# Arash-san/YinYang-Game-AlphaZero

Measured on AMD Instinct MI355X. Metric: self-play positions/sec (+ MCTS node-expansions/sec) at 800 sims, 8x8 board, higher is better.
Workload: dtype f16x3; 1 GPU; 8x8 board, 800 sims/move, 4096 concurrent games per GPU, frozen random-init 128x10 net (seed 0), copied boards, reference_quirks=False, staggered start plies; tree_arithmetic=f32 PUCT + u64 bitboards, nn_dtype=f16x3, evaluation_reuse=False, parallelism=episode-sharded x1, lanes_per_gpu=2, hipgraph=True

## Files before the change

include/yy_engine.h:

```cpp
#ifndef YY_ENGINE_H
#define YY_ENGINE_H

#include <stdint.h>

#ifdef __cplusplus
extern "C" {
#endif

#define YY_OK 0
#define YY_E_INVALID (-1)
#define YY_E_UNSUPPORTED (-2)
#define YY_E_NOMEM (-3)
#define YY_E_HIP (-4)
#define YY_E_STATE (-5)
#define YY_E_ARENA (-6)

#define YY_FLAG_ROWCOL 1u
#define YY_FLAG_ALIASED 2u
#define YY_FLAG_REUSE_PASS_VALUE 4u

#define YY_FLAG_REUSE_TRANSPOSITIONS 8u
#define YY_FLAG_KEEP_EVALUATIONS 16u

#define YY_FLAG_EVAL_SYMMETRY 32u
// ... 125 lines not shown
int yy_nn_tower_heads_bf16(const float *planes, const void *weights, const float *bias,
                           void *out_heads, int G, int R, int C, int channels, int n_layers,
                           yy_stream_t stream);

int yy_nn_tower_f32(const float *planes, const void *weights, const float *bias, float *out, int G,
                    int R, int C, int channels, int n_layers, yy_stream_t stream);

int yy_nn_head_finish_bf16(const void *h, int G, int A, int H, const float *w2, const float *b2,
                           float *policy, float *value, yy_stream_t stream);

int yy_nn_tower_f16x3_regs(const float *planes, const void *weights, const void *head_w, const float *bias,
                           float *out, float *out_heads, const int32_t *rows, const int32_t *n_rows, int G,
                           int R, int C, int channels, int n_layers, int weight_exp, int head_exp,
                           int act_exp, yy_stream_t stream);

int yy_nn_tower_g(const float *planes, const void *weights, const void *head_w, const float *bias, const float *head_bias,
                  float *out, float *out_heads, const int32_t *rows, const int32_t *n_rows, int G, int R, int C,
                  int channels, int n_layers, int weight_exp, int head_exp, int act_exp, int nb, int boards, int gate_lo,
                  int gate_hi, int layout, yy_stream_t stream);
int yy_nn_tower_g_forms(int channels, int *nb_out);
int yy_nn_tower_g_relu_check(uint32_t start, uint32_t count, uint32_t *counts, yy_stream_t stream);

int yy_nn_fc_heads_f16x3(const float *feats, const void *wpk, const float *bias, const int32_t *jobs, int n_jobs,
                         float *logits, float *hidden, const int32_t *n_rows, int G, int K, int A, int H,
                         int weight_exp, int act_exp, yy_stream_t stream);

int yy_nn_head_finish_f32(const float *logits, const float *hidden, int G, int A, int H, const float *w2,
                          const float *b2, const int32_t *rows, const int32_t *n_rows, float *policy,
                          float *value, yy_stream_t stream);

int yy_compact_rows(const uint8_t *flags, int G, int32_t *rows, int32_t *n, yy_stream_t stream);

int yy_selfplay_root_noise(uint64_t seed, const int64_t *game_id, const int32_t *ply, const uint8_t *draw,
                           const uint8_t *mask, int G, int A, double alpha, double *noise, yy_stream_t stream);

int yy_selfplay_root_gumbel(uint64_t seed, const int64_t *game_id, const int32_t *ply, int G, int A, float *rows,
                            yy_stream_t stream);

int yy_selfplay_sample_actions(uint64_t seed, const int64_t *game_id, const int32_t *ply,
                               const uint8_t *searching, const double *pi, const uint8_t *mask, int G, int A,
// ... 35 lines not shown
```

yinyang-game-alphazero_amd/_lib.py:

```python
import ctypes as C
import os
import subprocess

_HERE = os.path.dirname(os.path.abspath(__file__))
CSRC = os.path.join(_HERE, "csrc")
SO = os.path.join(CSRC, "libyy_hip.so")
HEADER = os.path.normpath(os.path.join(_HERE, "..", "include", "yy_engine.h"))

YY_OK = 0
YY_E_ARENA = -6
FLAG_ROWCOL = 1
FLAG_ALIASED = 2
FLAG_REUSE_PASS_VALUE = 4
FLAG_REUSE_TRANSPOSITIONS = 8
FLAG_KEEP_EVALUATIONS = 16
FLAG_EVAL_SYMMETRY = 32
FLAG_FORCED_PLAYOUTS = 64
FLAG_FPU_REDUCTION = 128
FLAG_SOLVER = 256
FLAG_GUMBEL_ROOT = 512
FLAG_GUMBEL_INTERIOR = 1024

HIPCC_FLAGS = ["--offload-arch=gfx950", "-O3", "-std=c++17", "-fPIC", "-shared",
               "-ffp-contract=off", "-fno-fast-math", "-Wall", "-Wno-unused-function"]
# ... 89 lines not shown
    "yy_mcts_shared_counters_ex": [_vp, C.POINTER(C.c_uint64)],
    "yy_nn_bias_act_bf16": [_vp, _vp, _vp, C.c_int64, C.c_int, C.c_int, _vp],
    "yy_nn_tower_bf16": [_vp, _vp, _vp, _vp, C.c_int, C.c_int, C.c_int, C.c_int, C.c_int, _vp],
    "yy_nn_tower_heads_bf16": [_vp, _vp, _vp, _vp, C.c_int, C.c_int, C.c_int, C.c_int, C.c_int, _vp],
    "yy_nn_head_finish_bf16": [_vp, C.c_int, C.c_int, C.c_int, _vp, _vp, _vp, _vp, _vp],
    "yy_nn_tower_f32": [_vp, _vp, _vp, _vp, C.c_int, C.c_int, C.c_int, C.c_int, C.c_int, _vp],
    "yy_nn_head_finish_f32": [_vp, _vp, C.c_int, C.c_int, C.c_int, _vp, _vp, _vp, _vp, _vp, _vp, _vp],
    "yy_compact_rows": [_vp, C.c_int, _vp, _vp, _vp],
    "yy_nn_tower_f16x3_regs": [_vp, _vp, _vp, _vp, _vp, _vp, _vp, _vp, C.c_int, C.c_int, C.c_int, C.c_int, C.c_int, C.c_int, C.c_int,
                               C.c_int, _vp],
    "yy_nn_tower_g_forms": [C.c_int, C.POINTER(C.c_int)],
    "yy_nn_tower_g_relu_check": [C.c_uint32, C.c_uint32, _vp, _vp],
    "yy_nn_tower_g": [_vp, _vp, _vp, _vp, _vp, _vp, _vp, _vp, _vp, C.c_int, C.c_int, C.c_int, C.c_int, C.c_int, C.c_int, C.c_int,
                      C.c_int, C.c_int, C.c_int, C.c_int, C.c_int, C.c_int, _vp],
    "yy_nn_fc_heads_f16x3": [_vp, _vp, _vp, _vp, C.c_int, _vp, _vp, _vp, C.c_int, C.c_int, C.c_int, C.c_int, C.c_int, C.c_int, _vp],
    "yy_selfplay_root_noise": [C.c_uint64, _vp, _vp, _vp, _vp, C.c_int, C.c_int, C.c_double, _vp, _vp],
    "yy_selfplay_root_gumbel": [C.c_uint64, _vp, _vp, C.c_int, C.c_int, _vp, _vp],
    "yy_selfplay_sample_actions": [C.c_uint64, _vp, _vp, _vp, _vp, _vp, C.c_int, C.c_int, C.c_int, _vp, _vp],
    "yy_selfplay_draw_budgets": [C.c_uint64, _vp, _vp, _vp, C.c_int, C.c_double, C.c_int, C.c_int, _vp, _vp, _vp],
    "yy_selfplay_run_create": [_vp, C.POINTER(SelfPlayConfig), C.POINTER(_vp)],
    "yy_selfplay_run_destroy": [_vp],
    "yy_selfplay_run_arm": [_vp, _vp, C.c_int64, C.c_int64, C.c_int64, _vp, _vp, _vp],
    "yy_mcts_step_selfplay": [_vp, _vp, _vp, _vp, _vp, _vp, _vp],
    "yy_selfplay_run_counters": [_vp, _vp, _vp],
    "yy_selfplay_run_examples": [_vp, C.c_int64, C.c_int64, _vp, _vp, _vp, _vp, _vp, _vp],
    "yy_version": [],
}


def exported_symbols():
# ... 25 lines not shown
```

yinyang-game-alphazero_amd/csrc/yy_engine.hip:

```cpp
#include <hip/hip_runtime.h>
#include <math.h>
#include <stdio.h>
#include <string.h>

#include "../../include/yy_engine.h"
#include "yy_bitboard.h"
#include "yy_common.h"
#include "yy_tree.h"

#define YY_VERSION 111

static thread_local char g_err[512] = "";
static int set_err(int code, const char *fmt, const char *a = "", const char *b = "") {
    snprintf(g_err, sizeof g_err, fmt, a, b);
    return code;
}

extern "C" const char *yy_last_error(void) { return g_err; }
extern "C" int yy_tower_set_err(int code, const char *msg) { return set_err(code, "%s%s", msg); }
extern "C" int yy_version(void) { return YY_VERSION; }

static int check_geo(int G, int R, int C) {
    if (G <= 0 || R <= 0 || C <= 0) return set_err(YY_E_INVALID, "non-positive size%s%s");
    if (R > YY_MAX_DIM || C > YY_MAX_DIM || R * C > 64 * YY_MAX_NW)
        return set_err(YY_E_UNSUPPORTED, "board larger than 16x16 / 192 cells%s%s");
// ... 1932 lines not shown
```

yinyang-game-alphazero_amd/csrc/yy_fc_heads.hip:

```cpp
#include <hip/hip_runtime.h>
#include <math.h>
#include <stdint.h>

#include "../../include/yy_engine.h"

typedef __attribute__((ext_vector_type(8))) _Float16 f16x8;
typedef __attribute__((ext_vector_type(2))) _Float16 f16x2;
typedef __attribute__((ext_vector_type(4))) float f32x4;
typedef __attribute__((ext_vector_type(2))) float f32x2;
typedef __attribute__((ext_vector_type(4))) unsigned int u32x4;
typedef __attribute__((ext_vector_type(2))) unsigned int u32x2;

#include "yy_common.h"

namespace fch {

constexpr int KC = 128, RS = 288;

__device__ __forceinline__ void split_pair(const f32x2 a, uint32_t &hi, uint32_t &lo) {
    const f16x2 h = __builtin_convertvector(a, f16x2);
    const f32x2 r = a - __builtin_convertvector(h, f32x2);
    const f16x2 l = __builtin_convertvector(r, f16x2);
    hi = __builtin_bit_cast(uint32_t, h);
    lo = __builtin_bit_cast(uint32_t, l);
// ... 109 lines not shown
    const int o0 = job.out0 + wave * 16 + kg * 4;
    float b[4];
#pragma unroll
    for (int i = 0; i < 4; i++) b[i] = (o0 + i < job.out0 + job.nout) ? bias[boff + o0 + i] : 0.0f;
#pragma unroll
    for (int nb = 0; nb < NBR; nb++) {
        const int row = r0 + nb * 16 + n16;
        if (row < n_live) {
#pragma unroll
            for (int i = 0; i < 4; i++)
                if (o0 + i < job.out0 + job.nout) out[(size_t)row * W + o0 + i] = __builtin_fmaf(acc1[nb][i] + acc2[nb][i], out_scale, b[i]);
        }
    }
}

}

extern "C" int yy_nn_fc_heads_f16x3(const float *feats, const void *wpk, const float *bias, const int32_t *jobs, int n_jobs,
                                    float *logits, float *hidden, const int32_t *n_rows, int G, int K, int A, int H,
                                    int weight_exp, int act_exp, yy_stream_t s) {
    if (G == 0) return YY_OK;
    if (!feats || !wpk || !bias || !jobs || !logits || !hidden || G < 0 || n_jobs < 1 || K < 32 || (K & 31) || A < 1 || H < 1)
        return yy_tower_set_err(YY_E_INVALID, "yy_nn_fc_heads_f16x3: bad argument");
    const float in_scale = ldexpf(1.0f, act_exp), out_scale = ldexpf(1.0f, -(weight_exp + act_exp));
    if (G <= 2048)
        fch::k_fc_heads<32><<<dim3(((G + 31) / 32) * n_jobs), dim3(256), 0, (hipStream_t)s>>>(
            feats, (const unsigned char *)wpk, bias, (const fch::Job *)jobs, n_jobs, logits, hidden, n_rows, G, K, A, H, in_scale, out_scale);
    else
        fch::k_fc_heads<64><<<dim3(((G + 63) / 64) * n_jobs), dim3(256), 0, (hipStream_t)s>>>(
            feats, (const unsigned char *)wpk, bias, (const fch::Job *)jobs, n_jobs, logits, hidden, n_rows, G, K, A, H, in_scale, out_scale);
    if (hipGetLastError() != hipSuccess) return yy_tower_set_err(YY_E_HIP, "yy_nn_fc_heads_f16x3: launch failed");
    return YY_OK;
}
```

yinyang-game-alphazero_amd/csrc/yy_tower_g.hip:

```cpp
#include <hip/hip_runtime.h>
#include <math.h>
#include <stdint.h>

#include <type_traits>

#include "../../include/yy_engine.h"

typedef __attribute__((ext_vector_type(8))) _Float16 f16x8;
typedef __attribute__((ext_vector_type(2))) _Float16 f16x2;
typedef __attribute__((ext_vector_type(4))) float f32x4;
typedef __attribute__((ext_vector_type(2))) float f32x2;
typedef __attribute__((ext_vector_type(4))) unsigned int u32x4;
typedef __attribute__((ext_vector_type(2))) unsigned int u32x2;

#include "yy_common.h"

namespace tg {

template <int NW_, int NB_, int D_, bool RB_> struct Geo {
    static constexpr int NW = NW_, NB = NB_, D = D_, CH = 32 * NW_, NCOL = 16 * NB_;
    static constexpr bool RB = RB_;
    static constexpr int RS = (NW_ >= 3) ? 288 : 160;
    static constexpr int ZERO_OFF = NCOL * RS;
    static constexpr int PART_BYTES = ZERO_OFF + 512;
// ... 179 lines not shown
                                              u32x2 &hi, u32x2 &lo) {
    f32x4 v;
#pragma unroll
    for (int i = 0; i < 4; i++) v[i] = __builtin_fmaf(acc1[i] + acc2[i], acc_scale, bq[i]);
    if (CONV2) v += *(const f32x4 *)res;
#pragma unroll
    for (int i = 0; i < 4; i++) v[i] = RELU(v[i]);
    if (KEEP) *(f32x4 *)res = v;
    uint32_t h01, l01, h23, l23;
    split_pair((f32x2){v[0], v[1]}, h01, l01);
    split_pair((f32x2){v[2], v[3]}, h23, l23);
    hi = (u32x2){h01, h23};
    lo = (u32x2){l01, l23};
}

template <class GEO>
__device__ __forceinline__ void heads_tail(const unsigned char *lds, const unsigned char *head_w, const float *head_bias, float *out_heads,
                                           int g0, int n_live, int C, int cells, int TB, int lane, int wave, float head_scale) {
    constexpr int NW = GEO::NW, NB = GEO::NB, RS = GEO::RS;
    int lane2 = lane;
    asm volatile("" : "+v"(lane2));
    const int n16 = lane2 & 15, kg = lane2 >> 4;
    for (int hm = wave; hm < 4; hm += NW) {
        const int head = hm >> 1, mb = hm & 1;
        f16x8 wh[NW], wl[NW];
#pragma unroll
        for (int kq = 0; kq < NW; kq++) {
            const unsigned char *p = head_w + ((size_t)(hm * NW + kq) * 2) * 1024 + lane2 * 16;
            wh[kq] = __builtin_bit_cast(f16x8, *(const u32x4 *)p);
            wl[kq] = __builtin_bit_cast(f16x8, *(const u32x4 *)(p + 1024));
        }
        const float *hb = head_bias + head * 32 + mb * 16;
        float sb[16];
#pragma unroll
        for (int k = 0; k < 16; k++) {
            sb[k] = hb[k];
            asm volatile("" : "+s"(sb[k]));
        }
        f32x4 b;
#pragma unroll
        for (int i = 0; i < 4; i++) b[i] = kg == 0 ? sb[i] : kg == 1 ? sb[4 + i] : kg == 2 ? sb[8 + i] : sb[12 + i];
#pragma unroll
        for (int nb = 0; nb < NB; nb++) {
            const uint32_t xb = (uint32_t)((nb * 16 + n16) * RS + kg * 16);
            f32x4 h1 = {0.f, 0.f, 0.f, 0.f}, h2 = {0.f, 0.f, 0.f, 0.f};
#pragma unroll
            for (int kq = 0; kq < NW; kq++) {
                const f16x8 xh = __builtin_bit_cast(f16x8, *(const u32x4 *)(lds + xb + kq * 64));
                const f16x8 xl = __builtin_bit_cast(f16x8, *(const u32x4 *)(lds + xb + GEO::PART_BYTES + kq * 64));
                const f32x4 a = __builtin_amdgcn_mfma_f32_16x16x32_f16(wl[kq], xh, h2, 0, 0, 0);
                h1 = __builtin_amdgcn_mfma_f32_16x16x32_f16(wh[kq], xh, h1, 0, 0, 0);
                h2 = __builtin_amdgcn_mfma_f32_16x16x32_f16(wh[kq], xl, a, 0, 0, 0);
            }
            int bd, cell;
            col_board_cell<GEO>(nb * 16 + n16, C, cells, bd, cell);
            const int gb = g0 + bd;
            if (bd < TB && gb < n_live) {
                float *o = out_heads + (((size_t)gb * 2 + head) * 32 + mb * 16 + kg * 4) * cells + cell;
#pragma unroll
                for (int i = 0; i < 4; i++) o[i * cells] = relu_keep_nan(__builtin_fmaf(h1[i] + h2[i], head_scale, b[i]));
            }
        }
    }
}

template <class GEO>
__device__ __forceinline__ void store_activations(const unsigned char *lds, float *out, int g0, int n_live, int C, int cells, int TB,
                                                  float out_scale) {
    constexpr int CH = GEO::CH, RS = GEO::RS, NT = 64 * GEO::NW;
    const int ncol = TB * cells;
    for (int p = threadIdx.x; p < ncol * (CH / 4); p += NT) {
        const int col = p / (CH / 4), ch4 = p % (CH / 4);
        int b, cell;
        col_board_cell<GEO>(col, C, cells, b, cell);
        if (b < TB && g0 + b < n_live) {
            const u32x2 ph = *(const u32x2 *)(lds + col * RS + ch4 * 8);
            const u32x2 pl = *(const u32x2 *)(lds + GEO::PART_BYTES + col * RS + ch4 * 8);
            const f32x2 v01 = join_pair(ph.x, pl.x), v23 = join_pair(ph.y, pl.y);
            *(f32x4 *)(out + ((size_t)(g0 + b) * cells + cell) * CH + ch4 * 4) = (f32x4){v01.x, v01.y, v23.x, v23.y} * out_scale;
        }
    }
}

template <int NW_, int NB_, int D_, bool RB_>
__global__ void __launch_bounds__(64 * NW_, 1)
k_tower_g(const float *__restrict__ planes, const unsigned char *__restrict__ weights, const unsigned char *__restrict__ head_w,
          const float *__restrict__ bias, const float *__restrict__ head_bias, float *__restrict__ out, float *__restrict__ out_heads,
          const int *__restrict__ rows, const int *__restrict__ n_rows, int G, int R, int C, int TB, int n_layers, float in_scale,
          float acc_scale, float head_scale, float out_scale, int gate_lo, int gate_hi) {
    using GEO = Geo<NW_, NB_, D_, RB_>;
    constexpr int NW = GEO::NW, NB = GEO::NB, D = GEO::D, CH = GEO::CH, RS = GEO::RS;
    __shared__ __attribute__((aligned(256))) unsigned char lds[GEO::LDS_BYTES];
    const int n_live = n_rows ? min(*n_rows, G) : G;
    if (n_live <= gate_lo || n_live > gate_hi) return;
    const int g0 = blockIdx.x * TB;
    if (g0 >= n_live) return;
    const int lane = threadIdx.x & 63;
    const int wave = __builtin_amdgcn_readfirstlane(threadIdx.x >> 6);
    const int cells = R * C, n_tower = 9 + 9 * NW * (n_layers - 1), crs = (GEO::RB ? 16 : C) * RS;

    const uint32_t voff = (uint32_t)(wave * 4096 + lane * 16);
    WChunk<2> W[D];
// ... 38 lines not shown
        f32x4 acc1[NB][2], acc2[NB][2];
        __syncthreads();
        run_layer<GEO, true>(acc1, acc2, W, lds, weights, voff, chunk, n_tower, crs, geo);
        __syncthreads();
        epilogue(0, acc1, acc2, std::false_type{}, std::true_type{});
    }
    for (int L = 1; L < n_layers; L++) {
        f32x4 acc1[NB][2], acc2[NB][2];
        __syncthreads();
        run_layer<GEO, false>(acc1, acc2, W, lds, weights, voff, chunk, n_tower, crs, geo);
        __syncthreads();
        if ((L & 1) == 0) epilogue(L, acc1, acc2, std::true_type{}, std::true_type{});
        else epilogue(L, acc1, acc2, std::false_type{}, std::false_type{});
    }
    __syncthreads();
    if (out_heads) heads_tail<GEO>(lds, head_w, head_bias, out_heads, g0, n_live, C, cells, TB, lane, wave, head_scale);
    else store_activations<GEO>(lds, out, g0, n_live, C, cells, TB, out_scale);
}

template <int D_> struct Geo22 : Geo<4, 8, D_, true> {
    static constexpr int NBW = 4, MBW = 4;
    static constexpr int BIAS_OFF = Geo22::RES_OFF + Geo22::NW * MBW * NBW * 1024;
    static constexpr int LDS_BYTES = BIAS_OFF + 21 * Geo22::CH * 4;
    static_assert(LDS_BYTES <= 163840, "LDS layout");
};

__device__ __forceinline__ float relu_max(float v) { return __builtin_elementwise_maximum(v, 0.0f); }

template <int NH> constexpr bool off22(int tap, int b) { return (NH == 0 && b == 0 && tap < 3) || (NH == 1 && b == 3 && tap >= 6); }

struct Taps22 {
// ... 149 lines not shown
        epilogue(0, acc1, acc2, std::false_type{}, std::true_type{});
    }
    for (int L = 1; L < n_layers; L++) {
        f32x4 acc1[4][4], acc2[4][4];
        __syncthreads();
        run_layer22<GEO, NH, false>(acc1, acc2, W, lds, weights, voff, chunk, n_tower, t);
        __syncthreads();
        if ((L & 1) == 0) epilogue(L, acc1, acc2, std::true_type{}, std::true_type{});
        else epilogue(L, acc1, acc2, std::false_type{}, std::false_type{});
    }
}

template <int D_>
__global__ void __launch_bounds__(256, 1)
k_tower_g22(const float *__restrict__ planes, const unsigned char *__restrict__ weights, const unsigned char *__restrict__ head_w,
            const float *__restrict__ bias, const float *__restrict__ head_bias, float *__restrict__ out, float *__restrict__ out_heads,
            const int *__restrict__ rows, const int *__restrict__ n_rows, int G, int R, int C, int TB, int n_layers, float in_scale,
            float acc_scale, float head_scale, float out_scale, int gate_lo, int gate_hi) {
    using GEO = Geo22<D_>;
    __shared__ __attribute__((aligned(256))) unsigned char lds[GEO::LDS_BYTES];
    const int n_live = n_rows ? min(*n_rows, G) : G;
    if (n_live <= gate_lo || n_live > gate_hi) return;
    const int g0 = blockIdx.x * TB;
    if (g0 >= n_live) return;
    const int lane = threadIdx.x & 63, cells = R * C;
    const int wave = __builtin_amdgcn_readfirstlane(threadIdx.x >> 6);
    if (wave & 1) tower22<GEO, 1>(lds, planes, weights, bias, rows, g0, n_live, R, C, TB, n_layers, lane, wave, in_scale, acc_scale);
    else tower22<GEO, 0>(lds, planes, weights, bias, rows, g0, n_live, R, C, TB, n_layers, lane, wave, in_scale, acc_scale);
    __syncthreads();
    if (out_heads) heads_tail<GEO>(lds, head_w, head_bias, out_heads, g0, n_live, C, cells, TB, lane, wave, head_scale);
    else store_activations<GEO>(lds, out, g0, n_live, C, cells, TB, out_scale);
}

__global__ void __launch_bounds__(256) k_relu_check(uint32_t start, uint32_t count, uint32_t *counts) {
    for (uint64_t i = blockIdx.x * 256u + threadIdx.x; i < count; i += gridDim.x * 256u) {
        const uint32_t x = start + (uint32_t)i;
        float v = __builtin_bit_cast(float, x);
        asm volatile("" : "+v"(v));
        const float a = relu_keep_nan(v), b = relu_max(v);
        const bool ok = __builtin_isnan(v) ? __builtin_isnan(b) : __builtin_bit_cast(uint32_t, a) == __builtin_bit_cast(uint32_t, b);
        if (!ok) {
            atomicAdd(&counts[0], 1u);
            atomicMin(&counts[1], x);
        }
    }
// ... 52 lines not shown
        return 6;
    }
    if (channels == 32 || channels == 64 || channels == 96) {
        nb_out[0] = 4;
        nb_out[1] = 9;
        return 2;
    }
    return 0;
}

extern "C" int yy_nn_tower_g(const float *planes, const void *weights, const void *head_w, const float *bias, const float *head_bias,
                             float *out, float *out_heads, const int32_t *rows, const int32_t *n_rows, int G, int R, int C,
                             int channels, int n_layers, int weight_exp, int head_exp, int act_exp, int nb, int boards, int gate_lo,
                             int gate_hi, int layout, yy_stream_t s) {
    if (G == 0) return YY_OK;
    if (!planes || !weights || !bias || (!out && !out_heads) || (out_heads && (!head_w || !head_bias)) || G < 0 || (rows && !n_rows))
        return yy_tower_set_err(YY_E_INVALID, "yy_nn_tower_g: bad argument");
    if (R < 1 || C < 1 || R * C > 144 || channels < 32 || channels > 128 || (channels & 31) || n_layers < 1 || n_layers > 21 ||
        (n_layers & 1) == 0 || layout < 0 || layout > 2)
        return yy_tower_set_err(YY_E_UNSUPPORTED,
                                "yy_nn_tower_g: needs boards of at most 144 cells, 32/64/96/128 channels, at most 10 residual blocks");
    if (boards < 1 || nb < 1 || boards * R * C > 16 * nb) return yy_tower_set_err(YY_E_INVALID, "yy_nn_tower_g: boards * cells > 16 * nb");
    TgArgs a = {planes, weights, head_w, bias, head_bias, out, out_heads, rows, n_rows, G, R, C, boards, n_layers,
                {ldexpf(1.0f, act_exp), ldexpf(1.0f, -weight_exp), ldexpf(1.0f, -(head_exp + act_exp)), ldexpf(1.0f, -act_exp)},
                gate_lo, gate_hi, (hipStream_t)s};
    return dispatch_tg(channels / 32, nb, layout, a);
}

extern "C" int yy_nn_tower_g_relu_check(uint32_t start, uint32_t count, uint32_t *counts, yy_stream_t s) {
    if (!counts) return yy_tower_set_err(YY_E_INVALID, "yy_nn_tower_g_relu_check: bad argument");
    if (count == 0) return YY_OK;
    tg::k_relu_check<<<dim3(4096), dim3(256), 0, (hipStream_t)s>>>(start, count, counts);
    if (hipGetLastError() != hipSuccess) return yy_tower_set_err(YY_E_HIP, "yy_nn_tower_g_relu_check: launch failed");
    return YY_OK;
}
```

yinyang-game-alphazero_amd/engine.py:

```python
import ctypes as ct

import numpy as np
import torch

from . import _lib
from .options import SHARED_EVALUATIONS_DEFAULT_SLOTS, SHARED_EVALUATIONS_HIGH_WATER, forced_k, fpu_r, gumbel_m, shared_slots
from ._lib import FLAG_ALIASED, FLAG_EVAL_SYMMETRY, FLAG_FORCED_PLAYOUTS, FLAG_FPU_REDUCTION, FLAG_GUMBEL_INTERIOR, FLAG_GUMBEL_ROOT, FLAG_SOLVER, FLAG_REUSE_PASS_VALUE, FLAG_KEEP_EVALUATIONS, FLAG_REUSE_TRANSPOSITIONS, FLAG_ROWCOL, MctsConfig, check, lib


def _stream():
    return ct.c_void_p(torch.cuda.current_stream().cuda_stream)


def _p(t):
    return None if t is None else ct.c_void_p(t.data_ptr())


def _need(t, dtype, shape=None, name="tensor"):
    if not isinstance(t, torch.Tensor) or not t.is_cuda:
        raise _lib.YYError(-1, f"{name}: expected a ROCm device tensor (the hot path has no CPU fallback)")
    if t.dtype != dtype or not t.is_contiguous():
        raise _lib.YYError(-1, f"{name}: expected contiguous {dtype}, got {t.dtype} contiguous={t.is_contiguous()}")
    if shape is not None and tuple(t.shape) != tuple(shape):
        raise _lib.YYError(-1, f"{name}: expected shape {tuple(shape)}, got {tuple(t.shape)}")
# ... 164 lines not shown
    _need(weights, torch.int16, (9 + 36 * (n_layers - 1), 8192), "wave-major split-f16 tower weights")
    _need(bias, torch.float32, (n_layers, 128), "tower bias")
    out = torch.empty((G, R, Cc, 128), dtype=torch.float32, device=planes.device)
    with torch.cuda.device(planes.device):
        check(lib().yy_nn_tower_f16x3_regs(_p(planes), _p(weights), None, _p(bias), _p(out), None, None, None, G, R, Cc, 128, n_layers,
                                           int(exps[0]), 0, int(exps[2]), _stream()))
    return out.permute(0, 3, 1, 2)


def tower_g_available(channels):
    buf = (ct.c_int * 8)()
    n = lib().yy_nn_tower_g_forms(int(channels), buf)
    return [int(buf[i]) for i in range(n)]


def tower_g(planes, weights, bias, n_layers, exps, nb, boards, head_w=None, head_bias=None, rows=None, n_rows=None, out=None,
            gate=(-1, 0x7FFFFFFF), column_layout=False, wave_grid=True):
    G, _, R, Cc = planes.shape
    _need(planes, torch.float32, (G, 5, R, Cc), "planes")
    ch = bias.shape[1]
    nw = ch // 32
    _need(weights, torch.int16, (9 + 9 * nw * (n_layers - 1), ch * 64), "split-f16 tower weights (pack_tower_g)")
    _need(bias, torch.float32, (n_layers, ch), "tower bias")
    if rows is not None:
        _need(rows, torch.int32, (G,), "rows")
        _need(n_rows, torch.int32, (1,), "n_rows")
    heads = head_w is not None
    if heads:
        _need(head_w, torch.int16, (4 * nw * 2 * 512,), "split-f16 head weights (pack_heads_g)")
        _need(head_bias, torch.float32, (64,), "head bias")
        if out is None:
            out = torch.empty((G, 2, 32 * R * Cc), dtype=torch.float32, device=planes.device)
        _need(out, torch.float32, (G, 2, 32 * R * Cc), "out")
    else:
        out = torch.empty((G, R, Cc, ch), dtype=torch.float32, device=planes.device)
    with torch.cuda.device(planes.device):
        check(lib().yy_nn_tower_g(_p(planes), _p(weights), _p(head_w), _p(bias), _p(head_bias), None if heads else _p(out),
                                  _p(out) if heads else None, _p(rows), _p(n_rows), G, R, Cc, ch, n_layers, int(exps[0]), int(exps[1]),
                                  int(exps[2]), int(nb), int(boards), int(gate[0]), int(gate[1]),
                                  1 if column_layout else 0 if wave_grid else 2,
                                  _stream()))
    return out if heads else out.permute(0, 3, 1, 2)


def tower_g_relu_check(start, count, counts):
    _need(counts, torch.int32, (2,), "counts")
    with torch.cuda.device(counts.device):
        check(lib().yy_nn_tower_g_relu_check(int(start) & 0xFFFFFFFF, int(count), _p(counts), _stream()))
    return counts


def fc_heads(feats, wpk, bias, jobs, A, H, exps, n_rows=None, logits=None, hidden=None):
    G, two, K = feats.shape
    _need(feats, torch.float32, (G, 2, K), "feats")
    _need(jobs, torch.int32, (jobs.shape[0], 4), "jobs")
    ksteps = ((K + 127) // 128) * 4
    _need(wpk, torch.int16, (jobs.shape[0] * ksteps * 4096,), "fc head weights (pack_fc_heads)")
    _need(bias, torch.float32, (A + H,), "fc head bias")
    if n_rows is not None:
        _need(n_rows, torch.int32, (1,), "n_rows")
    if logits is None:
        logits = torch.empty((G, A), dtype=torch.float32, device=feats.device)
        hidden = torch.empty((G, H), dtype=torch.float32, device=feats.device)
    _need(logits, torch.float32, (G, A), "logits")
    _need(hidden, torch.float32, (G, H), "hidden")
    with torch.cuda.device(feats.device):
        check(lib().yy_nn_fc_heads_f16x3(_p(feats), _p(wpk), _p(bias), _p(jobs), jobs.shape[0], _p(logits), _p(hidden), _p(n_rows), G, K,
                                         A, H, int(exps[0]), int(exps[1]), _stream()))
    return logits, hidden


def head_finish_f32(logits, hidden, w2, b2, rows=None, n_rows=None, policy=None, value=None):
    G, A = logits.shape
    _need(logits, torch.float32, name="logits")
    _need(hidden, torch.float32, (G, hidden.shape[1]), "hidden")
    _need(w2, torch.float32, (hidden.shape[1],), "w2")
    _need(b2, torch.float32, (1,), "b2")
    if rows is not None:
        _need(rows, torch.int32, (G,), "rows")
        _need(n_rows, torch.int32, (1,), "n_rows")
    if policy is None:
        policy = torch.zeros((G, A), dtype=torch.float32, device=logits.device)
        value = torch.zeros(G, dtype=torch.float32, device=logits.device)
# ... 621 lines not shown
```

yinyang-game-alphazero_amd/network.py:

```python
import os

import numpy as np
import torch
import torch.nn as nn
import torch.nn.functional as F

from . import engine

H3_BOARDS = ((6, 6), (8, 8), (12, 12))
G_MAX_CELLS = 144
G_CHANNELS = (32, 64, 96, 128)
G_SPLIT_WG = 256
G_HINT_BIG_ONLY = 4
G_AUTO_MAX_WG = 2048
HEAD_CHANNELS = 32
VALUE_HIDDEN = 256
INPUT_PLANES = 5


class ResidualBlock(nn.Module):

    def __init__(self, channels):
        super().__init__()
        for i in (1, 2):
# ... 78 lines not shown

def fold_batchnorm(conv, bn):
    scale = bn.weight / torch.sqrt(bn.running_var + bn.eps)
    w = conv.weight * scale.reshape(-1, 1, 1, 1)
    b = (conv.bias - bn.running_mean) * scale + bn.bias
    return w.detach(), b.detach()


def tower_convs(net):
    convs = [(net.conv1, net.bn1)]
    for blk in net.res_blocks:
        convs += [(blk.conv1, blk.bn1), (blk.conv2, blk.bn2)]
    return convs


ACT_EXP = 3


def _pow2_exponent(t, target=14):
    m = float(t.abs().max())
    if not np.isfinite(m) or m <= 0.0:
        return 0
    return int(target - 1 - np.floor(np.log2(m)))


def split_f16(t):
    t = t.float()
    hi = t.to(torch.float16)
    if not bool(torch.isfinite(hi).all()):
        raise ValueError("split-f16 evaluator: a scaled weight exceeds the float16 range")
# ... 250 lines not shown
        if small == big or G > G_AUTO_MAX_WG * small[1]:
            return [(big, ungated)]
        if G <= split:
            return [(small, ungated)]
        if not compacted:
            return [(big, ungated)]
        hint = self._hint.get(owner) if owner is not True and owner is not False else None
        if hint is not None and hint >= G_HINT_BIG_ONLY * split:
            return [(big, ungated)]
        return [(small, (-1, split)), (big, (split, 0x7FFFFFFF))]

    def _forward_split_f16(self, planes, needs_eval, static):
        G = planes.shape[0]
        K = 32 * planes.shape[2] * planes.shape[3]
        rows = n = pol = val = feats = logits = hidden = None
        if static:
            key = (G, 0 if static is True else static)
            buf = self._static.get(key)
            if buf is None:
                dev = planes.device
                z = lambda shape, dt=torch.float32: torch.zeros(shape, dtype=dt, device=dev)
                buf = self._static[key] = (z(G, torch.int32), z(1, torch.int32), z((G, self.n_actions)), z(G), z((G, 2, K)),
                                         z((G, self.n_actions)), z((G, self.n_hidden)))
            rows, n, pol, val, feats, logits, hidden = buf
        if needs_eval is not None:
            rows, n = engine.compact_rows(needs_eval, rows, n)
        else:
            rows = n = None
        if self.use_h3r:
            feats = engine.tower_heads_forward_h3r(planes, self.h3r_w, self.h3r_hw, self.h3_b, self.h3_layers, self.h3_exps, rows, n, feats)
        else:
            for form, gate in self._form_plan(G, rows is not None, static):
                feats = engine.tower_g(planes, self.g_w, self.g_b, self.h3_layers, self.g_exps, form[0], form[1],
                                       self.g_hw, self.g_hb, rows, n, feats, gate)
        logits, hidden = engine.fc_heads(feats, self.fc_w, self.fc_b, self.fc_jobs, self.n_actions, self.n_hidden, self.fc_exps, n,
                                         logits, hidden)
        return engine.head_finish_f32(logits, hidden, self.fc2_w, self.fc2_b, rows, n, pol, val)

    def _forward_fp32(self, planes, needs_eval, static):
        return self.net.predict_batch(planes)

    def _init_fp32t(self, net):
        if tuple(net.board_size) != (8, 8) or net.conv1.out_channels != 128 or len(net.res_blocks) > 11:
            raise ValueError(self.mode + " needs 8x8 boards, 128 channels, at most 11 residual blocks")
        wq, bq = pack_tower_f32(net)
        self.f32_w, self.f32_b = wq.to(self.device), bq.to(self.device)
# ... 85 lines not shown
```

Before: 1715 positions/s.

## Emit head features pre-split into f16 hi/lo MFMA operand layout from tower kernel

The tower kernel's head epilogue can now stage head-conv outputs in LDS and write them directly as split f16 hi/lo pairs in the tiled layout the FC-heads MFMA consumes. A new FC-heads kernel reads that operand layout with a register ring prefetch and needs no per-element f32-to-f16 splitting. The path is taken for batches above 2048 rows. This removes an f32 round-trip and the conversion work in the FC stage, at the cost of an extra LDS staging pass and barrier in the tower tail and padded 16-row buffers.

Measured after the change: 1711 positions/s. No clear change (-0.2%).

```diff
diff --git a/include/yy_engine.h b/include/yy_engine.h
--- a/include/yy_engine.h
+++ b/include/yy_engine.h
@@ -163,6 +163,7 @@
                            int R, int C, int channels, int n_layers, int weight_exp, int head_exp,
                            int act_exp, yy_stream_t stream);
 
+#define YY_TOWER_G_SPLIT_HEADS 4
 int yy_nn_tower_g(const float *planes, const void *weights, const void *head_w, const float *bias, const float *head_bias,
                   float *out, float *out_heads, const int32_t *rows, const int32_t *n_rows, int G, int R, int C,
                   int channels, int n_layers, int weight_exp, int head_exp, int act_exp, int nb, int boards, int gate_lo,
@@ -173,6 +174,9 @@
 int yy_nn_fc_heads_f16x3(const float *feats, const void *wpk, const float *bias, const int32_t *jobs, int n_jobs,
                          float *logits, float *hidden, const int32_t *n_rows, int G, int K, int A, int H,
                          int weight_exp, int act_exp, yy_stream_t stream);
+int yy_nn_fc_heads_op_f16x3(const void *xop, const void *wpk, const float *bias, const int32_t *jobs, int n_jobs,
+                            float *logits, float *hidden, const int32_t *n_rows, int G, int K, int A, int H,
+                            int weight_exp, int act_exp, yy_stream_t stream);
 
 int yy_nn_head_finish_f32(const float *logits, const float *hidden, int G, int A, int H, const float *w2,
                           const float *b2, const int32_t *rows, const int32_t *n_rows, float *policy,
diff --git a/yinyang-game-alphazero_amd/_lib.py b/yinyang-game-alphazero_amd/_lib.py
--- a/yinyang-game-alphazero_amd/_lib.py
+++ b/yinyang-game-alphazero_amd/_lib.py
@@ -127,6 +127,7 @@
     "yy_nn_tower_g": [_vp, _vp, _vp, _vp, _vp, _vp, _vp, _vp, _vp, C.c_int, C.c_int, C.c_int, C.c_int, C.c_int, C.c_int, C.c_int,
                       C.c_int, C.c_int, C.c_int, C.c_int, C.c_int, C.c_int, _vp],
     "yy_nn_fc_heads_f16x3": [_vp, _vp, _vp, _vp, C.c_int, _vp, _vp, _vp, C.c_int, C.c_int, C.c_int, C.c_int, C.c_int, C.c_int, _vp],
+    "yy_nn_fc_heads_op_f16x3": [_vp, _vp, _vp, _vp, C.c_int, _vp, _vp, _vp, C.c_int, C.c_int, C.c_int, C.c_int, C.c_int, C.c_int, _vp],
     "yy_selfplay_root_noise": [C.c_uint64, _vp, _vp, _vp, _vp, C.c_int, C.c_int, C.c_double, _vp, _vp],
     "yy_selfplay_root_gumbel": [C.c_uint64, _vp, _vp, C.c_int, C.c_int, _vp, _vp],
     "yy_selfplay_sample_actions": [C.c_uint64, _vp, _vp, _vp, _vp, _vp, C.c_int, C.c_int, C.c_int, _vp, _vp],
diff --git a/yinyang-game-alphazero_amd/csrc/yy_engine.hip b/yinyang-game-alphazero_amd/csrc/yy_engine.hip
--- a/yinyang-game-alphazero_amd/csrc/yy_engine.hip
+++ b/yinyang-game-alphazero_amd/csrc/yy_engine.hip
@@ -8,7 +8,7 @@
 #include "yy_common.h"
 #include "yy_tree.h"
 
-#define YY_VERSION 111
+#define YY_VERSION 112
 
 static thread_local char g_err[512] = "";
 static int set_err(int code, const char *fmt, const char *a = "", const char *b = "") {
diff --git a/yinyang-game-alphazero_amd/csrc/yy_fc_heads.hip b/yinyang-game-alphazero_amd/csrc/yy_fc_heads.hip
--- a/yinyang-game-alphazero_amd/csrc/yy_fc_heads.hip
+++ b/yinyang-game-alphazero_amd/csrc/yy_fc_heads.hip
@@ -147,6 +147,117 @@
     }
 }
 
+template <int MB> struct OpStep {
+    f16x8 wh[MB], wl[MB], xh[2], xl[2];
+};
+
+template <int MB>
+__device__ __forceinline__ void fc_op_jobs(const unsigned char *const (&xb)[2], const unsigned char *__restrict__ wpk, const float *__restrict__ bias,
+                                           const Job *__restrict__ jobs, int j0, float *__restrict__ out, int W, int boff, int r0, int n_live,
+                                           int KS, float out_scale, int lane, int wave) {
+    constexpr int D = MB == 1 ? 6 : MB == 4 ? 3 : 4;
+    const int n16 = lane & 15, kg = lane >> 4;
+    Job job[MB];
+    uint32_t woff[MB];
+#pragma unroll
+    for (int m = 0; m < MB; m++) {
+        job[m] = jobs[j0 + m];
+        woff[m] = (uint32_t)job[m].wchunk * 8192u;
+    }
+    const uint32_t wv = (uint32_t)(wave * 2048 + lane * 16);
+    auto load = [&](OpStep<MB> &s, int ks) {
+#pragma unroll
+        for (int m = 0; m < MB; m++) {
+            const unsigned char *p = wpk + (woff[m] + (uint32_t)ks * 8192u) + wv;
+            s.wh[m] = __builtin_bit_cast(f16x8, *(const u32x4 *)p);
+            s.wl[m] = __builtin_bit_cast(f16x8, *(const u32x4 *)(p + 1024));
+        }
+#pragma unroll
+        for (int nb = 0; nb < 2; nb++) {
+            const unsigned char *q = xb[nb] + (size_t)ks * 2048;
+            s.xh[nb] = __builtin_bit_cast(f16x8, *(const u32x4 *)q);
+            s.xl[nb] = __builtin_bit_cast(f16x8, *(const u32x4 *)(q + 1024));
+        }
+    };
+    f32x4 acc1[MB][2], acc2[MB][2];
+#pragma unroll
+    for (int m = 0; m < MB; m++)
+#pragma unroll
+        for (int nb = 0; nb < 2; nb++) acc1[m][nb] = acc2[m][nb] = (f32x4){0.f, 0.f, 0.f, 0.f};
+    OpStep<MB> ring[D];
+#pragma unroll
+    for (int j = 0; j < D; j++) load(ring[j], min(j, KS - 1));
+    auto compute = [&](const OpStep<MB> &s) {
+#pragma unroll
+        for (int nb = 0; nb < 2; nb++)
+#pragma unroll
+            for (int m = 0; m < MB; m++) {
+                const f32x4 a = __builtin_amdgcn_mfma_f32_16x16x32_f16(s.wl[m], s.xh[nb], acc2[m][nb], 0, 0, 0);
+                acc1[m][nb] = __builtin_amdgcn_mfma_f32_16x16x32_f16(s.wh[m], s.xh[nb], acc1[m][nb], 0, 0, 0);
+                acc2[m][nb] = __builtin_amdgcn_mfma_f32_16x16x32_f16(s.wh[m], s.xl[nb], a, 0, 0, 0);
+            }
+    };
+    int k0 = 0;
+    for (; k0 + D <= KS; k0 += D) {
+#pragma unroll
+        for (int j = 0; j < D; j++) {
+            compute(ring[j]);
+            load(ring[j], min(k0 + j + D, KS - 1));
+        }
+    }
+#pragma unroll
+    for (int j = 0; j < D - 1; j++)
+        if (k0 + j < KS) compute(ring[j]);
+#pragma unroll
+    for (int m = 0; m < MB; m++) {
+        const int o0 = job[m].out0 + wave * 16 + kg * 4, oe = job[m].out0 + job[m].nout;
+        float b[4];
+#pragma unroll
+        for (int i = 0; i < 4; i++) b[i] = (o0 + i < oe) ? bias[boff + o0 + i] : 0.0f;
+#pragma unroll
+        for (int nb = 0; nb < 2; nb++) {
+            const int row = r0 + nb * 16 + n16;
+            if (row < n_live) {
+#pragma unroll
+                for (int i = 0; i < 4; i++)
+                    if (o0 + i < oe) out[(size_t)row * W + o0 + i] = __builtin_fmaf(acc1[m][nb][i] + acc2[m][nb][i], out_scale, b[i]);
+            }
+        }
+    }
+}
+
+__global__ void __launch_bounds__(256, 1)
+k_fc_heads_op(const unsigned char *__restrict__ xop, const unsigned char *__restrict__ wpk, const float *__restrict__ bias,
+              const Job *__restrict__ jobs, int n_jobs, float *__restrict__ logits, float *__restrict__ hidden,
+              const int *__restrict__ n_rows, int G, int KS, int A, int H, float out_scale) {
+    const int n_live = n_rows ? min(*n_rows, G) : G;
+    const int n_tiles = gridDim.x >> 1;
+    const int head = blockIdx.x < n_tiles ? 1 : 0;
+    const int r0 = (blockIdx.x - (head ? 0 : n_tiles)) * 32;
+    if (r0 >= n_live) return;
+    const int lane = threadIdx.x & 63, wave = __builtin_amdgcn_readfirstlane(threadIdx.x >> 6);
+    int j0 = 0, nj = 0;
+    for (int j = 0; j < n_jobs; j++)
+        if (jobs[j].head == head) {
+            if (nj == 0) j0 = j;
+            nj++;
+        }
+    const unsigned char *xb[2];
+#pragma unroll
+    for (int nb = 0; nb < 2; nb++) {
+        const int row = min(r0 + nb * 16 + (lane & 15), n_live - 1);
+        xb[nb] = xop + (((size_t)(row >> 4) * 2 + head) * KS) * 2048 + ((lane >> 4) * 16 + (row & 15)) * 16;
+    }
+    float *out = head == 0 ? logits : hidden;
+    const int W = head == 0 ? A : H, boff = head == 0 ? 0 : A;
+    for (; nj > 0; j0 += 4, nj -= 4) {
+        if (nj >= 4) fc_op_jobs<4>(xb, wpk, bias, jobs, j0, out, W, boff, r0, n_live, KS, out_scale, lane, wave);
+        else if (nj == 3) fc_op_jobs<3>(xb, wpk, bias, jobs, j0, out, W, boff, r0, n_live, KS, out_scale, lane, wave);
+        else if (nj == 2) fc_op_jobs<2>(xb, wpk, bias, jobs, j0, out, W, boff, r0, n_live, KS, out_scale, lane, wave);
+        else fc_op_jobs<1>(xb, wpk, bias, jobs, j0, out, W, boff, r0, n_live, KS, out_scale, lane, wave);
+    }
+}
+
 }
 
 extern "C" int yy_nn_fc_heads_f16x3(const float *feats, const void *wpk, const float *bias, const int32_t *jobs, int n_jobs,
@@ -165,3 +276,17 @@
     if (hipGetLastError() != hipSuccess) return yy_tower_set_err(YY_E_HIP, "yy_nn_fc_heads_f16x3: launch failed");
     return YY_OK;
 }
+
+extern "C" int yy_nn_fc_heads_op_f16x3(const void *xop, const void *wpk, const float *bias, const int32_t *jobs, int n_jobs,
+                                       float *logits, float *hidden, const int32_t *n_rows, int G, int K, int A, int H,
+                                       int weight_exp, int act_exp, yy_stream_t s) {
+    if (G == 0) return YY_OK;
+    if (!xop || !wpk || !bias || !jobs || !logits || !hidden || G < 0 || n_jobs < 1 || K < 32 || (K & 31) || A < 1 || H < 1)
+        return yy_tower_set_err(YY_E_INVALID, "yy_nn_fc_heads_op_f16x3: bad argument");
+    const float out_scale = ldexpf(1.0f, -(weight_exp + act_exp));
+    fch::k_fc_heads_op<<<dim3(((G + 31) / 32) * 2), dim3(256), 0, (hipStream_t)s>>>(
+        (const unsigned char *)xop, (const unsigned char *)wpk, bias, (const fch::Job *)jobs, n_jobs, logits, hidden, n_rows, G, K / 32, A, H,
+        out_scale);
+    if (hipGetLastError() != hipSuccess) return yy_tower_set_err(YY_E_HIP, "yy_nn_fc_heads_op_f16x3: launch failed");
+    return YY_OK;
+}
diff --git a/yinyang-game-alphazero_amd/csrc/yy_tower_g.hip b/yinyang-game-alphazero_amd/csrc/yy_tower_g.hip
--- a/yinyang-game-alphazero_amd/csrc/yy_tower_g.hip
+++ b/yinyang-game-alphazero_amd/csrc/yy_tower_g.hip
@@ -217,53 +217,96 @@
     lo = (u32x2){l01, l23};
 }
 
+template <class GEO, class EMIT>
+__device__ __forceinline__ void head_unit(const unsigned char *lds, const unsigned char *head_w, const float *head_bias, int hm, int lane2,
+                                          float head_scale, EMIT emit) {
+    constexpr int NW = GEO::NW, NB = GEO::NB, RS = GEO::RS;
+    const int n16 = lane2 & 15, kg = lane2 >> 4;
+    const int head = hm >> 1, mb = hm & 1;
+    f16x8 wh[NW], wl[NW];
+#pragma unroll
+    for (int kq = 0; kq < NW; kq++) {
+        const unsigned char *p = head_w + ((size_t)(hm * NW + kq) * 2) * 1024 + lane2 * 16;
+        wh[kq] = __builtin_bit_cast(f16x8, *(const u32x4 *)p);
+        wl[kq] = __builtin_bit_cast(f16x8, *(const u32x4 *)(p + 1024));
+    }
+    const float *hb = head_bias + head * 32 + mb * 16;
+    float sb[16];
+#pragma unroll
+    for (int k = 0; k < 16; k++) {
+        sb[k] = hb[k];
+        asm volatile("" : "+s"(sb[k]));
+    }
+    f32x4 b;
+#pragma unroll
+    for (int i = 0; i < 4; i++) b[i] = kg == 0 ? sb[i] : kg == 1 ? sb[4 + i] : kg == 2 ? sb[8 + i] : sb[12 + i];
+#pragma unroll
+    for (int nb = 0; nb < NB; nb++) {
+        const uint32_t xb = (uint32_t)((nb * 16 + n16) * RS + kg * 16);
+        f32x4 h1 = {0.f, 0.f, 0.f, 0.f}, h2 = {0.f, 0.f, 0.f, 0.f};
+#pragma unroll
+        for (int kq = 0; kq < NW; kq++) {
+            const f16x8 xh = __builtin_bit_cast(f16x8, *(const u32x4 *)(lds + xb + kq * 64));
+            const f16x8 xl = __builtin_bit_cast(f16x8, *(const u32x4 *)(lds + xb + GEO::PART_BYTES + kq * 64));
+            const f32x4 a = __builtin_amdgcn_mfma_f32_16x16x32_f16(wl[kq], xh, h2, 0, 0, 0);
+            h1 = __builtin_amdgcn_mfma_f32_16x16x32_f16(wh[kq], xh, h1, 0, 0, 0);
+            h2 = __builtin_amdgcn_mfma_f32_16x16x32_f16(wh[kq], xl, a, 0, 0, 0);
+        }
+        f32x4 v;
+#pragma unroll
+        for (int i = 0; i < 4; i++) v[i] = relu_keep_nan(__builtin_fmaf(h1[i] + h2[i], head_scale, b[i]));
+        emit(nb, v);
+    }
+}
+
 template <class GEO>
-__device__ __forceinline__ void heads_tail(const unsigned char *lds, const unsigned char *head_w, const float *head_bias, float *out_heads,
-                                           int g0, int n_live, int C, int cells, int TB, int lane, int wave, float head_scale) {
-    constexpr int NW = GEO::NW, NB = GEO::NB, RS = GEO::RS;
+__device__ __forceinline__ void heads_tail(unsigned char *lds, const unsigned char *head_w, const float *head_bias, float *out_heads,
+                                           bool split, int g0, int n_live, int C, int cells, int TB, int lane, int wave,
+                                           float head_scale, float in_scale) {
+    constexpr int NW = GEO::NW, NB = GEO::NB, NT = 64 * NW;
+    unsigned char *out_split = split ? (unsigned char *)out_heads : nullptr;
     int lane2 = lane;
     asm volatile("" : "+v"(lane2));
     const int n16 = lane2 & 15, kg = lane2 >> 4;
-    for (int hm = wave; hm < 4; hm += NW) {
-        const int head = hm >> 1, mb = hm & 1;
-        f16x8 wh[NW], wl[NW];
-#pragma unroll
-        for (int kq = 0; kq < NW; kq++) {
-            const unsigned char *p = head_w + ((size_t)(hm * NW + kq) * 2) * 1024 + lane2 * 16;
-            wh[kq] = __builtin_bit_cast(f16x8, *(const u32x4 *)p);
-            wl[kq] = __builtin_bit_cast(f16x8, *(const u32x4 *)(p + 1024));
-        }
-        const float *hb = head_bias + head * 32 + mb * 16;
-        float sb[16];
-#pragma unroll
-        for (int k = 0; k < 16; k++) {
-            sb[k] = hb[k];
-            asm volatile("" : "+s"(sb[k]));
-        }
-        f32x4 b;
-#pragma unroll
-        for (int i = 0; i < 4; i++) b[i] = kg == 0 ? sb[i] : kg == 1 ? sb[4 + i] : kg == 2 ? sb[8 + i] : sb[12 + i];
-#pragma unroll
-        for (int nb = 0; nb < NB; nb++) {
-            const uint32_t xb = (uint32_t)((nb * 16 + n16) * RS + kg * 16);
-            f32x4 h1 = {0.f, 0.f, 0.f, 0.f}, h2 = {0.f, 0.f, 0.f, 0.f};
-#pragma unroll
-            for (int kq = 0; kq < NW; kq++) {
-                const f16x8 xh = __builtin_bit_cast(f16x8, *(const u32x4 *)(lds + xb + kq * 64));
-                const f16x8 xl = __builtin_bit_cast(f16x8, *(const u32x4 *)(lds + xb + GEO::PART_BYTES + kq * 64));
-                const f32x4 a = __builtin_amdgcn_mfma_f32_16x16x32_f16(wl[kq], xh, h2, 0, 0, 0);
-                h1 = __builtin_amdgcn_mfma_f32_16x16x32_f16(wh[kq], xh, h1, 0, 0, 0);
-                h2 = __builtin_amdgcn_mfma_f32_16x16x32_f16(wh[kq], xl, a, 0, 0, 0);
-            }
-            int bd, cell;
-            col_board_cell<GEO>(nb * 16 + n16, C, cells, bd, cell);
-            const int gb = g0 + bd;
-            if (bd < TB && gb < n_live) {
-                float *o = out_heads + (((size_t)gb * 2 + head) * 32 + mb * 16 + kg * 4) * cells + cell;
-#pragma unroll
-                for (int i = 0; i < 4; i++) o[i * cells] = relu_keep_nan(__builtin_fmaf(h1[i] + h2[i], head_scale, b[i]));
-            }
-        }
+    constexpr int NP = NW == 1 ? 2 : 1, HP = 2 / NP;
+    static_assert(GEO::NCOL * HP * 128 <= NW * 2 * NB * 1024, "the staged features fit the residual's LDS");
+    float *stage = (float *)(lds + GEO::RES_OFF);
+    const int K = 32 * cells, live = min(TB, n_live - g0);
+    for (int ps = 0; ps < NP; ps++) {
+        for (int hm = ps * 2 * HP + wave; hm < (ps + 1) * 2 * HP; hm += NW) {
+            const int head = hm >> 1, mb = hm & 1;
+            head_unit<GEO>(lds, head_w, head_bias, hm, lane2, head_scale, [&](int nb, const f32x4 v) {
+                int bd, cell;
+                col_board_cell<GEO>(nb * 16 + n16, C, cells, bd, cell);
+                if (bd >= live) return;
+                if (out_split) {
+                    float *o = stage + ((bd * HP + head - ps * HP) * 32 + mb * 16 + kg * 4) * cells + cell;
+#pragma unroll
+                    for (int i = 0; i < 4; i++) o[i * cells] = v[i];
+                } else {
+                    float *o = out_heads + (((size_t)(g0 + bd) * 2 + head) * 32 + mb * 16 + kg * 4) * cells + cell;
+#pragma unroll
+                    for (int i = 0; i < 4; i++) o[i * cells] = v[i];
+                }
+            });
+        }
+        if (!out_split) continue;
+        __syncthreads();
+        for (int idx = threadIdx.x; idx < live * 4 * cells * HP; idx += NT) {
+            const int q = idx / live, bd = idx - q * live, kgo = q & 3, r = q >> 2, hl = r / cells, ks = r - hl * cells;
+            const float *src = stage + (bd * HP + hl) * K + ks * 32 + kgo * 8;
+            const f32x4 a = *(const f32x4 *)src * in_scale, b = *(const f32x4 *)(src + 4) * in_scale;
+            uint32_t h01, l01, h23, l23, h45, l45, h67, l67;
+            split_pair((f32x2){a[0], a[1]}, h01, l01);
+            split_pair((f32x2){a[2], a[3]}, h23, l23);
+            split_pair((f32x2){b[0], b[1]}, h45, l45);
+            split_pair((f32x2){b[2], b[3]}, h67, l67);
+            const int row = g0 + bd;
+            unsigned char *dst = out_split + ((((size_t)(row >> 4) * 2 + ps * HP + hl) * cells + ks) * 128 + kgo * 16 + (row & 15)) * 16;
+            *(u32x4 *)dst = (u32x4){h01, h23, h45, h67};
+            *(u32x4 *)(dst + 1024) = (u32x4){l01, l23, l45, l67};
+        }
+        if (ps + 1 < NP) __syncthreads();
     }
 }
 
@@ -288,7 +331,7 @@
 template <int NW_, int NB_, int D_, bool RB_>
 __global__ void __launch_bounds__(64 * NW_, 1)
 k_tower_g(const float *__restrict__ planes, const unsigned char *__restrict__ weights, const unsigned char *__restrict__ head_w,
-          const float *__restrict__ bias, const float *__restrict__ head_bias, float *__restrict__ out, float *__restrict__ out_heads,
+          const float *__restrict__ bias, const float *__restrict__ head_bias, float *out, float *out_heads,
           const int *__restrict__ rows, const int *__restrict__ n_rows, int G, int R, int C, int TB, int n_layers, float in_scale,
           float acc_scale, float head_scale, float out_scale, int gate_lo, int gate_hi) {
     using GEO = Geo<NW_, NB_, D_, RB_>;
@@ -357,7 +400,7 @@
         else epilogue(L, acc1, acc2, std::false_type{}, std::false_type{});
     }
     __syncthreads();
-    if (out_heads) heads_tail<GEO>(lds, head_w, head_bias, out_heads, g0, n_live, C, cells, TB, lane, wave, head_scale);
+    if (out_heads) heads_tail<GEO>(lds, head_w, head_bias, out_heads, out == out_heads, g0, n_live, C, cells, TB, lane, wave, head_scale, 1.0f / out_scale);
     else store_activations<GEO>(lds, out, g0, n_live, C, cells, TB, out_scale);
 }
 
@@ -537,7 +580,7 @@
 template <int D_>
 __global__ void __launch_bounds__(256, 1)
 k_tower_g22(const float *__restrict__ planes, const unsigned char *__restrict__ weights, const unsigned char *__restrict__ head_w,
-            const float *__restrict__ bias, const float *__restrict__ head_bias, float *__restrict__ out, float *__restrict__ out_heads,
+            const float *__restrict__ bias, const float *__restrict__ head_bias, float *out, float *out_heads,
             const int *__restrict__ rows, const int *__restrict__ n_rows, int G, int R, int C, int TB, int n_layers, float in_scale,
             float acc_scale, float head_scale, float out_scale, int gate_lo, int gate_hi) {
     using GEO = Geo22<D_>;
@@ -551,7 +594,7 @@
     if (wave & 1) tower22<GEO, 1>(lds, planes, weights, bias, rows, g0, n_live, R, C, TB, n_layers, lane, wave, in_scale, acc_scale);
     else tower22<GEO, 0>(lds, planes, weights, bias, rows, g0, n_live, R, C, TB, n_layers, lane, wave, in_scale, acc_scale);
     __syncthreads();
-    if (out_heads) heads_tail<GEO>(lds, head_w, head_bias, out_heads, g0, n_live, C, cells, TB, lane, wave, head_scale);
+    if (out_heads) heads_tail<GEO>(lds, head_w, head_bias, out_heads, out == out_heads, g0, n_live, C, cells, TB, lane, wave, head_scale, 1.0f / out_scale);
     else store_activations<GEO>(lds, out, g0, n_live, C, cells, TB, out_scale);
 }
 
@@ -634,17 +677,18 @@
                              int channels, int n_layers, int weight_exp, int head_exp, int act_exp, int nb, int boards, int gate_lo,
                              int gate_hi, int layout, yy_stream_t s) {
     if (G == 0) return YY_OK;
+    const bool split = layout >= 0 && (layout & YY_TOWER_G_SPLIT_HEADS);
     if (!planes || !weights || !bias || (!out && !out_heads) || (out_heads && (!head_w || !head_bias)) || G < 0 || (rows && !n_rows))
         return yy_tower_set_err(YY_E_INVALID, "yy_nn_tower_g: bad argument");
     if (R < 1 || C < 1 || R * C > 144 || channels < 32 || channels > 128 || (channels & 31) || n_layers < 1 || n_layers > 21 ||
-        (n_layers & 1) == 0 || layout < 0 || layout > 2)
+        (n_layers & 1) == 0 || layout < 0 || (layout & 3) > 2 || layout > 7 || (split && !out_heads))
         return yy_tower_set_err(YY_E_UNSUPPORTED,
                                 "yy_nn_tower_g: needs boards of at most 144 cells, 32/64/96/128 channels, at most 10 residual blocks");
     if (boards < 1 || nb < 1 || boards * R * C > 16 * nb) return yy_tower_set_err(YY_E_INVALID, "yy_nn_tower_g: boards * cells > 16 * nb");
-    TgArgs a = {planes, weights, head_w, bias, head_bias, out, out_heads, rows, n_rows, G, R, C, boards, n_layers,
+    TgArgs a = {planes, weights, head_w, bias, head_bias, split ? out_heads : out, out_heads, rows, n_rows, G, R, C, boards, n_layers,
                 {ldexpf(1.0f, act_exp), ldexpf(1.0f, -weight_exp), ldexpf(1.0f, -(head_exp + act_exp)), ldexpf(1.0f, -act_exp)},
                 gate_lo, gate_hi, (hipStream_t)s};
-    return dispatch_tg(channels / 32, nb, layout, a);
+    return dispatch_tg(channels / 32, nb, layout & 3, a);
 }
 
 extern "C" int yy_nn_tower_g_relu_check(uint32_t start, uint32_t count, uint32_t *counts, yy_stream_t s) {
diff --git a/yinyang-game-alphazero_amd/engine.py b/yinyang-game-alphazero_amd/engine.py
--- a/yinyang-game-alphazero_amd/engine.py
+++ b/yinyang-game-alphazero_amd/engine.py
@@ -202,8 +202,20 @@
     return [int(buf[i]) for i in range(n)]
 
 
+def split_heads_buffer(G, cells, device, zero=False):
+    make = torch.zeros if zero else torch.empty
+    return make(((G + 15) // 16 * 16, 2, 64 * cells), dtype=torch.int16, device=device)[:G]
+
+
+def _need_split_heads(t, G, cells, name):
+    _need(t, torch.int16, (G, 2, 64 * cells), name)
+    if (t.untyped_storage().nbytes() - t.storage_offset() * 2) < (G + 15) // 16 * 16 * 256 * cells or t.storage_offset() % 8:
+        raise _lib.YYError(-1, f"{name}: the storage must cover whole 16-row blocks (engine.split_heads_buffer)")
+    return t
+
+
 def tower_g(planes, weights, bias, n_layers, exps, nb, boards, head_w=None, head_bias=None, rows=None, n_rows=None, out=None,
-            gate=(-1, 0x7FFFFFFF), column_layout=False, wave_grid=True):
+            gate=(-1, 0x7FFFFFFF), column_layout=False, wave_grid=True, split_heads=False):
     G, _, R, Cc = planes.shape
     _need(planes, torch.float32, (G, 5, R, Cc), "planes")
     ch = bias.shape[1]
@@ -217,16 +229,24 @@
     if heads:
         _need(head_w, torch.int16, (4 * nw * 2 * 512,), "split-f16 head weights (pack_heads_g)")
         _need(head_bias, torch.float32, (64,), "head bias")
-        if out is None:
-            out = torch.empty((G, 2, 32 * R * Cc), dtype=torch.float32, device=planes.device)
-        _need(out, torch.float32, (G, 2, 32 * R * Cc), "out")
+        split_heads = split_heads or (out is not None and out.dtype == torch.int16)
+        if split_heads:
+            if out is None:
+                out = split_heads_buffer(G, R * Cc, planes.device)
+            _need_split_heads(out, G, R * Cc, "out (split head features)")
+        else:
+            if out is None:
+                out = torch.empty((G, 2, 32 * R * Cc), dtype=torch.float32, device=planes.device)
+            _need(out, torch.float32, (G, 2, 32 * R * Cc), "out")
     else:
+        if split_heads:
+            raise ValueError("tower_g: split_heads needs the head convolutions (head_w, head_bias)")
         out = torch.empty((G, R, Cc, ch), dtype=torch.float32, device=planes.device)
     with torch.cuda.device(planes.device):
         check(lib().yy_nn_tower_g(_p(planes), _p(weights), _p(head_w), _p(bias), _p(head_bias), None if heads else _p(out),
                                   _p(out) if heads else None, _p(rows), _p(n_rows), G, R, Cc, ch, n_layers, int(exps[0]), int(exps[1]),
                                   int(exps[2]), int(nb), int(boards), int(gate[0]), int(gate[1]),
-                                  1 if column_layout else 0 if wave_grid else 2,
+                                  (1 if column_layout else 0 if wave_grid else 2) + (4 if split_heads else 0),
                                   _stream()))
     return out if heads else out.permute(0, 3, 1, 2)
 
@@ -239,6 +259,8 @@
 
 
 def fc_heads(feats, wpk, bias, jobs, A, H, exps, n_rows=None, logits=None, hidden=None):
+    if feats.dtype == torch.int16:
+        return fc_heads_op(feats, wpk, bias, jobs, A, H, exps, n_rows, logits, hidden)
     G, two, K = feats.shape
     _need(feats, torch.float32, (G, 2, K), "feats")
     _need(jobs, torch.int32, (jobs.shape[0], 4), "jobs")
@@ -255,6 +277,27 @@
     with torch.cuda.device(feats.device):
         check(lib().yy_nn_fc_heads_f16x3(_p(feats), _p(wpk), _p(bias), _p(jobs), jobs.shape[0], _p(logits), _p(hidden), _p(n_rows), G, K,
                                          A, H, int(exps[0]), int(exps[1]), _stream()))
+    return logits, hidden
+
+
+def fc_heads_op(xop, wpk, bias, jobs, A, H, exps, n_rows=None, logits=None, hidden=None):
+    G, _, k2 = xop.shape
+    K = k2 // 2
+    _need_split_heads(xop, G, K // 32, "xop")
+    _need(jobs, torch.int32, (jobs.shape[0], 4), "jobs")
+    ksteps = ((K + 127) // 128) * 4
+    _need(wpk, torch.int16, (jobs.shape[0] * ksteps * 4096,), "fc head weights (pack_fc_heads)")
+    _need(bias, torch.float32, (A + H,), "fc head bias")
+    if n_rows is not None:
+        _need(n_rows, torch.int32, (1,), "n_rows")
+    if logits is None:
+        logits = torch.empty((G, A), dtype=torch.float32, device=xop.device)
+        hidden = torch.empty((G, H), dtype=torch.float32, device=xop.device)
+    _need(logits, torch.float32, (G, A), "logits")
+    _need(hidden, torch.float32, (G, H), "hidden")
+    with torch.cuda.device(xop.device):
+        check(lib().yy_nn_fc_heads_op_f16x3(_p(xop), _p(wpk), _p(bias), _p(jobs), jobs.shape[0], _p(logits), _p(hidden), _p(n_rows), G, K,
+                                            A, H, int(exps[0]), int(exps[1]), _stream()))
     return logits, hidden
 
 
diff --git a/yinyang-game-alphazero_amd/network.py b/yinyang-game-alphazero_amd/network.py
--- a/yinyang-game-alphazero_amd/network.py
+++ b/yinyang-game-alphazero_amd/network.py
@@ -116,6 +116,7 @@
     return convs
 
 
+FC_OPERAND_ABOVE = 2048
 ACT_EXP = 3
 
 
@@ -396,13 +397,16 @@
         G = planes.shape[0]
         K = 32 * planes.shape[2] * planes.shape[3]
         rows = n = pol = val = feats = logits = hidden = None
+        cells = planes.shape[2] * planes.shape[3]
         if static:
             key = (G, 0 if static is True else static)
             buf = self._static.get(key)
             if buf is None:
                 dev = planes.device
                 z = lambda shape, dt=torch.float32: torch.zeros(shape, dtype=dt, device=dev)
-                buf = self._static[key] = (z(G, torch.int32), z(1, torch.int32), z((G, self.n_actions)), z(G), z((G, 2, K)),
+                buf = self._static[key] = (z(G, torch.int32), z(1, torch.int32), z((G, self.n_actions)), z(G),
+                                         engine.split_heads_buffer(G, cells, dev, zero=True) if G > FC_OPERAND_ABOVE and not self.use_h3r
+                                         else z((G, 2, K)),
                                          z((G, self.n_actions)), z((G, self.n_hidden)))
             rows, n, pol, val, feats, logits, hidden = buf
         if needs_eval is not None:
@@ -412,6 +416,8 @@
         if self.use_h3r:
             feats = engine.tower_heads_forward_h3r(planes, self.h3r_w, self.h3r_hw, self.h3_b, self.h3_layers, self.h3_exps, rows, n, feats)
         else:
+            if feats is None and G > FC_OPERAND_ABOVE:
+                feats = engine.split_heads_buffer(G, cells, planes.device)
             for form, gate in self._form_plan(G, rows is not None, static):
                 feats = engine.tower_g(planes, self.g_w, self.g_b, self.h3_layers, self.g_exps, form[0], form[1],
                                        self.g_hw, self.g_hb, rows, n, feats, gate)
```
